# nfrasser/lasgun

Hardware: NVIDIA B200
Metric: Mrays/s (primary+shadow) (higher is better)
Workload: dtype f64

## Files before the change

lasgun_b200/csrc/lgb_kernels.cu:

```cuda
#include <math_constants.h>

#include <algorithm>

#include "lgb_math.cuh"

namespace lgb {

template <class T> __device__ __forceinline__ void wst(T* p, T v) { __stcs(p, v); }
template <class T> __device__ __forceinline__ T wld(const T* p) { return __ldcs(p); }

struct RayF {
    float ox, oy, oz;
    float ix, iy, iz;
    float nx, ny, nz;
    float dx, dy, dz;
    float inv_dd, inv_len;
    float sx, sy, sz;
    float err;
    int kz;
    unsigned oct;
};

__device__ __forceinline__ float clamp_idir(float d) {
    const float v = 1.0f / d;
// ... 1286 lines not shown
        const unsigned long long v0 = __popc(__ballot_sync(0xFFFFFFFFu, primary != 0)), v1 = __popc(__ballot_sync(0xFFFFFFFFu, hits != 0));
        if (lane == 0) { atomicAdd(&ctr(O)->primary_rays, v0); atomicAdd(&ctr(O)->primary_hits, v1); }
        if (STATS) {
            for (int k = 0; k < 3; k++) {
                unsigned long long a = warp_sum(lc.filter[k]), b = warp_sum(lc.exact[k]);
                if (lane == 0) { atomicAdd(&ctr(O)->filter[k], a); atomicAdd(&ctr(O)->exact[k], b); atomicAdd(&ctr(O)->p_filter[k], a); atomicAdd(&ctr(O)->p_exact[k], b); }
            }
        }
    }
}

template <bool ALL_SHADOWS, bool INST, bool RAYBUF = false>
__global__ void __launch_bounds__(kAppendThreads) k_setup(DevScene S, DevCamera C, DevShade sh, DevWork W, DevOut O, DevWave V) {
    constexpr bool LEAN = !INST && !RAYBUF;
    const uint64_t total = W.n_pixels * W.spp;
    const uint64_t g = (uint64_t)blockIdx.x * blockDim.x + threadIdx.x;
    uint32_t need = 0;
    bool live = false;
    if (g < total) {
        const uint32_t ref = V.hit_ref[g];
        const double t_hit = V.hit_t[g];
        Ray64 ray; uint32_t x, y, s;
        bool ref_done = false;
        if (ref != kSlotUnused && slot_ray<RAYBUF>(C, W, g, ray, x, y, s)) {
            const uint64_t gi = ((uint64_t)y * W.w + x) * W.spp + s;
            if (ref == LGB_MISS) {
                if (O.aov_id) O.aov_id[gi] = LGB_MISS;
                if (O.aov_t) O.aov_t[gi] = CUDART_INF;
                if (O.aov_occl) O.aov_occl[gi] = 0;
            } else {
                if (!ALL_SHADOWS && S.specular && (material_flags(S, ref) & kMatSpecular)) { V.occl[g] = 0; V.gate[g] = 0; ref_done = true; }
            }
            if (ref != LGB_MISS && !ref_done) {
                live = true;
                const double t = t_hit;
                D3 ng, ps; double wo_ng; uint32_t sflags = kSfGeneric;
                if (LEAN) {
                    LeanSurf Ls;
                    lean_surface<true>(S, ray, t, ref, 0u, Ls);
                    sflags = Ls.flags;
                    if (!(sflags & kSfGeneric)) {
                        ng = (sflags & kSfNgFlip) ? -Ls.n : Ls.n;
                        ps = ray.o + ray.d * t + ng * (2.220446049250313e-16 * 65536.0);
                        wo_ng = 1.0;
                    }
                }
                if (sflags & kSfGeneric) {
                    ShadePoint P; uint32_t id;
                    shade_point<false, INST>(S, ray, t, ref, P, id);
                    ng = P.ng; ps = P.ps; wo_ng = dot(P.wo, P.ng);
                }
                V.ps[3 * g + 0] = ps.x; V.ps[3 * g + 1] = ps.y; V.ps[3 * g + 2] = ps.z;
                if (O.aov_id) O.aov_id[gi] = canonical_id(S, ref);
                if (O.aov_t) O.aov_t[gi] = t;
                const uint32_t gate = light_gates(S, ray, ps, ng, wo_ng, !(sflags & kSfGeneric));
                need = ALL_SHADOWS ? (S.n_lights >= 32u ? 0xFFFFFFFFu : (1u << S.n_lights) - 1u) : gate;
                V.occl[g] = 0;
                V.gate[g] = gate;
                if (LEAN) V.sflags[g] = (unsigned char)sflags;
            }
        }
    }
    if (S.grids) return;
    __shared__ MultiAppendScratch sc;
    __shared__ uint32_t qmap[2 * LGB_MAX_LIGHTS];
    if (threadIdx.x < 2 * S.n_lights) qmap[threadIdx.x] = (threadIdx.x >> 1) * 3 + ((threadIdx.x & 1) ? kQueueB : kQueueA);
    __syncthreads();
    const bool anchor = W.spp == 1 || (uint32_t)g - fdiv((uint32_t)g, W.fd_spp) * W.spp == W.anchor;
    unsigned long long flags = 0;
    if (live) for (uint32_t l = 0; l < S.n_lights; l++) if ((need >> l) & 1u) flags |= 1ull << (2 * l + (anchor ? 0 : 1));
    block_append_multi(sc, 2 * S.n_lights, flags, (uint32_t)g, V.queue, V.queue_stride, V.queue_count, qmap);
}

template <bool INST>
__device__ __forceinline__ bool occludes(const DevScene& S, uint32_t ref, const Ray64& world) {
    const uint32_t type = ref >> 30, idx = ref & 0x3FFFFFFFu;
    Ray64 ray = world;
    if (INST) ray = ray_to_space(S, space_of(S, ref), world);
    double t;
    if (type == LGB_PRIM_TRIANGLE) {
        const float4* tp = S.tri + 3 * (size_t)idx;
        const float4 q0 = __ldg(tp), q1 = __ldg(tp + 1), q2 = __ldg(tp + 2);
        double b0, b1, b2;
        return triangle_exact(d3(q0.x, q0.y, q0.z), d3(q1.x, q1.y, q1.z), d3(q2.x, q2.y, q2.z), ray, t, b0, b1, b2) && t < 1.0;
    }
    if (type == LGB_PRIM_SPHERE) {
        const double2 c01 = __ldg(reinterpret_cast<const double2*>(S.sph64 + 4 * (size_t)idx));
        const double2 c23 = __ldg(reinterpret_cast<const double2*>(S.sph64 + 4 * (size_t)idx + 2));
        bool inside;
        return sphere_exact(d3(c01.x, c01.y, c23.x), c23.y, ray, t, inside) && t < 1.0;
    }
    double mn[3], mx[3];
#pragma unroll
    for (int k = 0; k < 3; k++) { mn[k] = __ldg(&S.cub64[6 * (size_t)idx + k]); mx[k] = __ldg(&S.cub64[6 * (size_t)idx + 3 + k]); }
    int ua, va;
    return cuboid_exact(mn, mx, ray, t, ua, va) && t < 1.0;
}

#ifndef LGB_PRETEST_ITEMS
#define LGB_PRETEST_ITEMS 2
#endif
constexpr int kPretestItems = LGB_PRETEST_ITEMS;
template <bool INST>
__global__ void __launch_bounds__(kAppendThreads) k_pretest(DevScene S, DevWork W, DevOut O, DevWave V, uint32_t light) {
    __shared__ AppendScratch sc;
    const unsigned total = V.queue_count[light * 3 + kQueueB];
    const unsigned lane = threadIdx.x & 31u;
    const double* L = S.lights + 9 * (size_t)light;
    const D3 lp = d3(L[0], L[1], L[2]);
    unsigned ncached = 0;
    for (uint64_t i0 = (uint64_t)blockIdx.x * blockDim.x * kPretestItems; i0 < total; i0 += (uint64_t)gridDim.x * blockDim.x * kPretestItems) {
        const uint64_t first = i0 + threadIdx.x * kPretestItems;
        uint32_t g[kPretestItems], oc[kPretestItems];
        unsigned to_c = 0;
#pragma unroll
        for (int k = 0; k < kPretestItems; k++) {
            g[k] = 0; oc[k] = LGB_MISS;
            if (first + k < total) {
                g[k] = V.queue[(size_t)(light * 3 + kQueueB) * V.queue_stride + first + k];
                if (g[k] != kEntryDone) {
                    oc[k] = V.occluder[(size_t)light * W.n_pixels + fdiv(g[k], W.fd_spp)];
                    to_c |= 1u << k;
                }
            }
        }
#pragma unroll
        for (int k = 0; k < kPretestItems; k++) {
            if (oc[k] != LGB_MISS) {
                Ray64 ray;
                ray.o = d3(V.ps[3 * (size_t)g[k]], V.ps[3 * (size_t)g[k] + 1], V.ps[3 * (size_t)g[k] + 2]);
                ray.d = lp - ray.o;
                if (occludes<INST>(S, oc[k], ray)) { atomicOr(&V.occl[g[k]], 1u << light); to_c &= ~(1u << k); ncached++; }
            }
        }
        block_append_n<kPretestItems>(sc, to_c, g, V.queue + (size_t)(light * 3 + kQueueC) * V.queue_stride, &V.queue_count[light * 3 + kQueueC]);
    }
    if (O.counters) {
        const unsigned long long n = warp_sum(ncached);
        if (lane == 0 && n) { atomicAdd(&ctr(O)->shadow_cached, n); atomicAdd(&ctr(O)->shadow_occluded, n); }
        if (blockIdx.x == 0 && threadIdx.x == 0) atomicAdd(&ctr(O)->shadow_traced, (unsigned long long)total);
    }
}

#ifndef LGB_SBEAM_THREADS
#define LGB_SBEAM_THREADS_ 64
#else
#define LGB_SBEAM_THREADS_ LGB_SBEAM_THREADS
#endif
template <bool STATS>
__global__ void __launch_bounds__(LGB_SBEAM_THREADS_, 1024 / LGB_SBEAM_THREADS_) k_sbeam(DevScene S, DevWork W, DevOut O, DevWave V, uint32_t light,
                                                                                     uint2* list_out, uint32_t* count_out) {
    const unsigned total = V.free_count[light];
    const unsigned i = blockIdx.x * blockDim.x + threadIdx.x;
    const unsigned lane = threadIdx.x & 31u;
    LocalCounters lc = {};
    if (i < total) {
        const uint32_t ga = V.queue[(size_t)(light * 3 + kQueueC) * V.queue_stride + i];
        const uint32_t p = fdiv(ga, W.fd_spp);
        {
        const double* Lp = S.lights + 9 * (size_t)light;
        const D3 lp = d3(Lp[0], Lp[1], Lp[2]);
        Ray64 centre; centre.o = lp;
        centre.d = d3(V.ps[3 * (size_t)ga], V.ps[3 * (size_t)ga + 1], V.ps[3 * (size_t)ga + 2]) - lp;
        double dmin[3] = {centre.d.x, centre.d.y, centre.d.z}, dmax[3] = {centre.d.x, centre.d.y, centre.d.z};
        for (uint32_t k = 0; k < W.spp; k++) {
            const size_t g = (size_t)p * W.spp + k;
            const uint32_t ref = V.hit_ref[g];
            if (ref == LGB_MISS || ref == kSlotUnused) continue;
            const double dx = V.ps[3 * g] - lp.x, dy = V.ps[3 * g + 1] - lp.y, dz = V.ps[3 * g + 2] - lp.z;
            dmin[0] = fmin(dmin[0], dx); dmax[0] = fmax(dmax[0], dx); dmin[1] = fmin(dmin[1], dy); dmax[1] = fmax(dmax[1], dy);
            dmin[2] = fmin(dmin[2], dz); dmax[2] = fmax(dmax[2], dz);
        }
        const double dc[3] = {centre.d.x, centre.d.y, centre.d.z};
        float sp[3];
        for (int a = 0; a < 3; a++) {
            if (!(dmin[a] > 0.0) && !(dmax[a] < 0.0)) { sp[a] = 1e30f; continue; }
            const double lo = fmin(fabs(dmin[a]), fabs(dmax[a])), hi = fmax(fabs(dmin[a]), fabs(dmax[a])), c = fabs(dc[a]);
            const double up = c / lo - 1.0, dn = 1.0 - c / hi;
            sp[a] = __double2float_ru(fmax(fmax(up, dn), 0.0) * 1.0000001 + 4e-7);
        }
        BeamF B; B.sx = sp[0]; B.sy = sp[1]; B.sz = sp[2];
        const RayF f = make_rayf(centre, S.err_abs);
        const float smax = 1.0f + 1e-5f;
        uint32_t stack[kStackDepth]; int sp_ = 0;
        uint2 list[kBeamList];
        uint32_t n = 0, cur = 0;
        bool over = false;
        while (cur != kDone && !over) {
            if (cur & kLeafBit) {
                const uint32_t type = (cur >> 29) & 3u, count = ((cur >> 24) & 31u) + 1u, first = cur & kLeafFirstMask;
                for (uint32_t k = 0; k < count; k++) {
                    const uint32_t idx = first + k;
                    float lx, ly, lz, hx, hy, hz;
                    if (type == LGB_PRIM_TRIANGLE) {
                        const float4* tp = S.tri + 3 * (size_t)idx;
                        const float4 q0 = __ldg(tp), q1 = __ldg(tp + 1), q2 = __ldg(tp + 2);
                        lx = fminf(q0.x, fminf(q1.x, q2.x)); hx = fmaxf(q0.x, fmaxf(q1.x, q2.x));
                        ly = fminf(q0.y, fminf(q1.y, q2.y)); hy = fmaxf(q0.y, fmaxf(q1.y, q2.y));
                        lz = fminf(q0.z, fminf(q1.z, q2.z)); hz = fmaxf(q0.z, fmaxf(q1.z, q2.z));
                    } else if (type == LGB_PRIM_SPHERE) {
                        const float4 s4 = __ldg(&S.sph32[idx]);
                        const float rr = __fadd_ru(s4.w, f.err);
                        lx = __fsub_rd(s4.x, rr); hx = __fadd_ru(s4.x, rr); ly = __fsub_rd(s4.y, rr); hy = __fadd_ru(s4.y, rr); lz = __fsub_rd(s4.z, rr); hz = __fadd_ru(s4.z, rr);
                    } else {
                        const float4 lo = __ldg(&S.cub32[2 * idx]), hi = __ldg(&S.cub32[2 * idx + 1]);
                        lx = lo.x; ly = lo.y; lz = lo.z; hx = hi.x; hy = hi.y; hz = hi.z;
                    }
                    if (type != LGB_PRIM_CUBOID) {
                        lx = __fsub_rd(lx, f.err); ly = __fsub_rd(ly, f.err); lz = __fsub_rd(lz, f.err);
                        hx = __fadd_ru(hx, f.err); hy = __fadd_ru(hy, f.err); hz = __fadd_ru(hz, f.err);
                    }
                    float tn;
                    if (!beam_slab<8>(lx, ly, lz, hx, hy, hz, f, B, tn) || tn > smax) continue;
                    if (n == (uint32_t)kBeamList) { over = true; break; }
                    list[n++] = make_uint2(kLeafBit | (type << 29) | idx, __float_as_uint(tn));
                }
                cur = kDone;
            } else {
                const float4* np = S.nodes + 4 * (size_t)cur;
                const float4 n0 = __ldg(np), n1 = __ldg(np + 1), n2 = __ldg(np + 2);
                const float2 n3 = __ldg(reinterpret_cast<const float2*>(np + 3));
                if (STATS) lc.node_tests++;
                float t0, t1;
                bool h0, h1;
                switch (f.oct) {
#define LGB_BEAM_CASE(o) case o: h0 = beam_slab<o>(n0.x, n0.y, n0.z, n0.w, n1.x, n1.y, f, B, t0); h1 = beam_slab<o>(n1.z, n1.w, n2.x, n2.y, n2.z, n2.w, f, B, t1); break;
                LGB_BEAM_CASE(0) LGB_BEAM_CASE(1) LGB_BEAM_CASE(2) LGB_BEAM_CASE(3) LGB_BEAM_CASE(4) LGB_BEAM_CASE(5) LGB_BEAM_CASE(6)
                default: h0 = beam_slab<7>(n0.x, n0.y, n0.z, n0.w, n1.x, n1.y, f, B, t0); h1 = beam_slab<7>(n1.z, n1.w, n2.x, n2.y, n2.z, n2.w, f, B, t1); break;
#undef LGB_BEAM_CASE
                }
                h0 = h0 && t0 <= smax; h1 = h1 && t1 <= smax;
                const uint32_t c0 = __float_as_uint(n3.x), c1 = __float_as_uint(n3.y);
                if (h0 && h1) { cur = c0; stack[sp_++] = c1; }
                else if (h0) cur = c0;
                else if (h1) cur = c1;
                else cur = kDone;
            }
            if (cur == kDone && sp_ && !over) cur = stack[--sp_];
        }
        if (!over) {
            for (uint32_t k = 0; k < n; k++) list_out[(size_t)k * W.n_pixels + p] = list[k];
            count_out[p] = n;
        }
        }
    }
    if (O.counters && STATS) {
        unsigned long long nt = warp_sum(lc.node_tests);
        if (lane == 0) atomicAdd(&ctr(O)->node_tests, nt);
    }
}
#ifndef LGB_SWALK_THREADS
#define LGB_SWALK_THREADS 128
#endif
#ifndef LGB_SBEAM_THREADS
#define LGB_SBEAM_THREADS 64
#endif
template <bool STATS>
__global__ void __launch_bounds__(LGB_SWALK_THREADS, 1024 / LGB_SWALK_THREADS) k_swalk(DevScene S, DevWork W, DevOut O, DevWave V, uint32_t light,
                                                                                       const uint2* list_in, const uint32_t* count_in) {
    const unsigned total = V.queue_count[light * 3 + kQueueB];
    const unsigned i = blockIdx.x * blockDim.x + threadIdx.x;
    const unsigned lane = threadIdx.x & 31u;
    LocalCounters lc = {};
    unsigned occluded = 0;
    if (i < total) {
        uint32_t* slot = V.queue + (size_t)(light * 3 + kQueueB) * V.queue_stride + i;
        const uint32_t g = *slot;
        const uint32_t p = fdiv(g, W.fd_spp);
        const uint32_t n = count_in[p];
        if (n != kBeamOverflow) {
            const double* Lp = S.lights + 9 * (size_t)light;
            Ray64 world;
            world.o = d3(V.ps[3 * (size_t)g], V.ps[3 * (size_t)g + 1], V.ps[3 * (size_t)g + 2]);
            world.d = d3(Lp[0], Lp[1], Lp[2]) - world.o;
            Ray64 ray; RayF f; Trav T;
            enter_root<false>(S, world, ray, f, T, 1.0);
            bool hit = false;
            for (uint32_t k = 0; k < n && !hit; k++) {
                const uint2 e = __ldg(&list_in[(size_t)k * W.n_pixels + p]);
                hit = leaf_prims<true, STATS, false>(S, world, ray, f, T, (e.x >> 29) & 3u, 1u, e.x & kLeafFirstMask, 1.0, lc);
            }
            if (hit) { atomicOr(&V.occl[g], 1u << light); occluded++; }
            *slot = kEntryDone;
        }
    }
    if (O.counters) {
        unsigned long long v = warp_sum(occluded);
        if (lane == 0 && v) atomicAdd(&ctr(O)->shadow_occluded, v);
        if (STATS) {
            for (int k = 0; k < 3; k++) {
                unsigned long long a = warp_sum(lc.filter[k]), b = warp_sum(lc.exact[k]);
                if (lane == 0) { atomicAdd(&ctr(O)->filter[k], a); atomicAdd(&ctr(O)->exact[k], b); }
            }
        }
    }
}

#ifndef LGB_GSHADOW_THREADS
#define LGB_GSHADOW_THREADS 64
#endif
#ifndef LGB_GSHADOW_MIN_BLOCKS
#define LGB_GSHADOW_MIN_BLOCKS (1536 / LGB_GSHADOW_THREADS)
#endif
template <bool STATS>
__device__ __forceinline__ bool grid_blocked(const DevScene& S, D3 o, uint32_t l, LocalCounters& lc) {
    Ray64 world;
    world.o = o;
    const double* Lp = S.lights + 9 * (size_t)l;
    world.d = d3(Lp[0], Lp[1], Lp[2]) - world.o;
    const double ax = fabs(world.d.x), ay = fabs(world.d.y), az = fabs(world.d.z);
    const int a = ax >= ay ? (ax >= az ? 0 : 2) : (ay >= az ? 1 : 2);
    const double da = -(a == 0 ? world.d.x : a == 1 ? world.d.y : world.d.z);
    const double db = -(a == 0 ? world.d.y : a == 1 ? world.d.z : world.d.x), dc = -(a == 0 ? world.d.z : a == 1 ? world.d.x : world.d.y);
    if (da == 0.0) return false;
    const DevGrid* G = S.grids + l;
    const uint32_t res = __ldg(&G->res), n_large = __ldg(&G->n_large);
    const int face = 2 * a + (da < 0.0 ? 1 : 0);
    const double* map = G->map[face];
    const double inv = fast_rcp(fabs(da));
    const int cu = min(max((int)floor((db * inv - __ldg(map)) * __ldg(map + 1)), 0), (int)res - 1);
    const int cv = min(max((int)floor((dc * inv - __ldg(map + 2)) * __ldg(map + 3)), 0), (int)res - 1);
    const size_t cell = ((size_t)face * res + (size_t)cv) * res + (size_t)cu;
    const uint32_t* cs = G->cell_start;
    const uint32_t b = __ldg(cs + cell), e = __ldg(cs + cell + 1);
    Ray64 ray; RayF f; Trav T;
    enter_root<false>(S, world, ray, f, T, 1.0);
    const float dd = f.dx * f.dx + f.dy * f.dy + f.dz * f.dz;
    const float len_up = dd * f.inv_len * (1.0f + 1e-5f) + f.err;
    bool hit = false;
    const bool sorted = e - b <= kGridSortMax;
    const uint2* en = G->entries;
    const uint2* lg = G->large;
    for (uint32_t i = b; i < e && !hit; i++) {
        const uint2 r = __ldg(en + i);
        if (__uint_as_float(r.y) > len_up) { if (sorted) break; else continue; }
        hit = leaf_prims<true, STATS, false>(S, world, ray, f, T, r.x >> 30, 1u, r.x & 0x3FFFFFFFu, 1.0, lc);
    }
    for (uint32_t i = 0; i < n_large && !hit; i++) {
        const uint2 r = __ldg(lg + i);
        if (__uint_as_float(r.y) > len_up) break;
        hit = leaf_prims<true, STATS, false>(S, world, ray, f, T, r.x >> 30, 1u, r.x & 0x3FFFFFFFu, 1.0, lc);
    }
    return hit;
}

template <bool STATS, bool ALL_SHADOWS>
__global__ void __launch_bounds__(LGB_GSHADOW_THREADS, LGB_GSHADOW_MIN_BLOCKS) k_gshadow(DevScene S, DevCamera C, DevWork W, DevOut O, DevWave V) {
    const uint64_t total = W.n_pixels * W.spp;
    const uint64_t g = (uint64_t)blockIdx.x * blockDim.x + threadIdx.x;
    const unsigned lane = threadIdx.x & 31u;
    LocalCounters lc = {};
    unsigned traced = 0, occluded = 0;
    if (g < total) {
        const uint32_t ref = wld(&V.hit_ref[g]);
        uint32_t mask = 0;
        D3 ps = d3(0, 0, 0);
        const uint32_t gate = ALL_SHADOWS ? (S.n_lights >= 32u ? 0xFFFFFFFFu : (1u << S.n_lights) - 1u) : wld(&V.gate[g]);
        ps = d3(wld(&V.ps[3 * g]), wld(&V.ps[3 * g + 1]), wld(&V.ps[3 * g + 2]));
        if (ref != LGB_MISS && ref != kSlotUnused) mask = gate;
        if (mask) {
            uint32_t occl = 0;
            for (uint32_t l = 0; l < S.n_lights; l++) {
                if (!((mask >> l) & 1u)) continue;
                traced++;
                if (grid_blocked<STATS>(S, ps, l, lc)) { occl |= 1u << l; occluded++; }
            }
            wst(&V.occl[g], occl);
        }
    }
    if (O.counters) {
        const unsigned long long v0 = warp_sum(traced), v1 = warp_sum(occluded);
        if (lane == 0 && v0) {
            if (W.mode == 3) atomicAdd(&ctr(O)->secondary_rays, v0);
            else { atomicAdd(&ctr(O)->shadow_traced, v0); atomicAdd(&ctr(O)->shadow_occluded, v1); }
        }
        if (STATS) {
            for (int k = 0; k < 3; k++) {
                unsigned long long a = warp_sum(lc.filter[k]), b = warp_sum(lc.exact[k]);
                if (lane == 0) { atomicAdd(&ctr(O)->filter[k], a); atomicAdd(&ctr(O)->exact[k], b); }
            }
        }
    }
}

template <bool STATS, bool INST>
__global__ void __launch_bounds__(LGB_TRAV_THREADS, LGB_MIN_BLOCKS) k_shadow(DevScene S, DevWork W, DevOut O, DevWave V, uint32_t light, int which) {
    const unsigned total = V.queue_count[light * 3 + which];
    const uint32_t* q = V.queue + (size_t)(light * 3 + which) * V.queue_stride;
    const bool record = which == kQueueA && W.spp > 1;
    const double* L = S.lights + 9 * (size_t)light;
    const D3 lp = d3(L[0], L[1], L[2]);
    const unsigned lane = threadIdx.x & 31u;
    LocalCounters lc = {};
    unsigned int occluded = 0;
    uint32_t stack[kStackDepth];
    Ray64 world, ray; RayF f; Trav T;
    uint32_t g = 0;
    bool active = false, drained = false;
    for (;;) {
        if (!drained) {
            const unsigned idle = __ballot_sync(0xFFFFFFFFu, !active);
            if (idle == 0xFFFFFFFFu) {
                const unsigned long long idx = warp_fetch(V.queue_fetch + light * 3 + which, !active, lane);
                if (!active && idx < total) {
                    g = q[idx];
                    world.o = d3(V.ps[3 * (size_t)g], V.ps[3 * (size_t)g + 1], V.ps[3 * (size_t)g + 2]);
                    world.d = lp - world.o;
                    enter_root<INST>(S, world, ray, f, T, 1.0); active = true;
                }
                drained = __any_sync(0xFFFFFFFFu, idx != ~0ull && idx >= total);
            }
        }
        const unsigned amask = __ballot_sync(0xFFFFFFFFu, active);
        if (!amask) break;
        const unsigned oct0 = __shfl_sync(0xFFFFFFFFu, f.oct, __ffs(amask) - 1);
        const unsigned octw = __all_sync(0xFFFFFFFFu, !active || f.oct == oct0) ? oct0 : 8u;
        if (active) {
            const bool done = trav_run<true, STATS, true, INST>(S, world, ray, f, T, stack, nullptr, 1.0, lc, 0, octw);
            if (done) {
                if (T.best.ref != LGB_MISS) { atomicOr(&V.occl[g], 1u << light); occluded++; }
                if (record) V.occluder[(size_t)light * W.n_pixels + fdiv(g, W.fd_spp)] = T.best.ref;
                if (record && W.beams && T.best.ref == LGB_MISS) {
                    const unsigned peers = __activemask(), leader = __ffs(peers) - 1;
                    uint32_t base = 0;
                    if (lane == leader) base = atomicAdd(V.free_count + light, (uint32_t)__popc(peers));
                    base = __shfl_sync(peers, base, leader);
                    V.queue[(size_t)(light * 3 + kQueueC) * V.queue_stride + base + __popc(peers & ((1u << lane) - 1u))] = g;
                }
                active = false;
            }
        }
    }
    if (O.counters) {
        unsigned long long v = warp_sum(occluded);
        if (lane == 0) atomicAdd(&ctr(O)->shadow_occluded, v);
        if (which == kQueueA && blockIdx.x == 0 && threadIdx.x == 0) atomicAdd(&ctr(O)->shadow_traced, (unsigned long long)total);
        if (STATS) {
            unsigned long long n = warp_sum(lc.node_tests);
            if (lane == 0) atomicAdd(&ctr(O)->node_tests, n);
            for (int k = 0; k < 3; k++) {
                unsigned long long a = warp_sum(lc.filter[k]), b = warp_sum(lc.exact[k]);
                if (lane == 0) { atomicAdd(&ctr(O)->filter[k], a); atomicAdd(&ctr(O)->exact[k], b); }
            }
        }
    }
}

#ifndef LGB_SHADE_MIN_BLOCKS
#define LGB_SHADE_MIN_BLOCKS 4
#endif
#ifndef LGB_FUSED_THREADS
#define LGB_FUSED_THREADS 128u
#endif
#ifndef LGB_GSHADE_MIN_BLOCKS
#define LGB_GSHADE_MIN_BLOCKS 2
#endif
__device__ __forceinline__ uchar4 quantise(D3 c) {
    uchar4 px;
    px.x = (unsigned char)round(fmin(fmax(c.x, 0.0), 1.0) * 255.0);
    px.y = (unsigned char)round(fmin(fmax(c.y, 0.0), 1.0) * 255.0);
    px.z = (unsigned char)round(fmin(fmax(c.z, 0.0), 1.0) * 255.0);
    px.w = 255;
    return px;
}
__device__ __forceinline__ void spawn_children(const ShadePoint& P, const DevWave& V, uint32_t g) {
    SpawnRec rec; rec.slot = g; rec.child_r = rec.child_t = kNoChild; rec.pad = 0;
    rec.spec_r[0] = rec.spec_r[1] = rec.spec_r[2] = rec.spec_t[0] = rec.spec_t[1] = rec.spec_t[2] = rec.c = 0.0;
    Ray64 rr, rt; D3 spec, wi;
    bool has_r = false, has_t = false;
    if (sample_specular_reflection(P.B, spec, wi) && !(spec.x == 0.0 && spec.y == 0.0 && spec.z == 0.0) && !(dot(wi, P.ns) <= 0.0)) {
        has_r = true; rr.o = P.ps; rr.d = -1.0 * P.wo + 2.0 * dot(P.wo, P.ns) * P.ns;
        rec.spec_r[0] = spec.x; rec.spec_r[1] = spec.y; rec.spec_r[2] = spec.z;
    }
    if (sample_specular_transmission(P.B, spec, wi)) {
        const double c = fabs(dot(wi, P.ns));
        if (!(spec.x == 0.0 && spec.y == 0.0 && spec.z == 0.0) && c != 0.0) {
            has_t = true; rt.o = P.pt; rt.d = wi; rec.c = c;
            rec.spec_t[0] = spec.x; rec.spec_t[1] = spec.y; rec.spec_t[2] = spec.z;
        }
    }
    const unsigned peers = __activemask(), lane = threadIdx.x & 31u, leader = __ffs(peers) - 1;
    const unsigned mr = __ballot_sync(peers, has_r), mt = __ballot_sync(peers, has_t);
    uint32_t b_rec = 0, b_r = 0, b_t = 0;
    if (lane == leader) {
        b_rec = atomicAdd(V.spawn_ctr, (uint32_t)__popc(peers));
        if (mr) b_r = atomicAdd(V.spawn_ctr + 1, (uint32_t)__popc(mr));
        if (mt) b_t = atomicAdd(V.spawn_ctr + 2, (uint32_t)__popc(mt));
    }
    b_rec = __shfl_sync(peers, b_rec, leader); b_r = __shfl_sync(peers, b_r, leader); b_t = __shfl_sync(peers, b_t, leader);
    const unsigned below = (1u << lane) - 1u;
    if (has_r) {
        rec.child_r = b_r + __popc(mr & below);
        double* o = V.next_rays + 6 * (size_t)rec.child_r; o[0] = rr.o.x; o[1] = rr.o.y; o[2] = rr.o.z; o[3] = rr.d.x; o[4] = rr.d.y; o[5] = rr.d.z;
    }
    if (has_t) {
        rec.child_t = V.next_t_base + b_t + __popc(mt & below);
        double* o = V.next_rays + 6 * (size_t)rec.child_t; o[0] = rt.o.x; o[1] = rt.o.y; o[2] = rt.o.z; o[3] = rt.d.x; o[4] = rt.d.y; o[5] = rt.d.z;
    }
    V.recs[b_rec + __popc(peers & below)] = rec;
}

template <bool INST, bool FUSED, bool GENERAL = false, bool RAYBUF = false>
__global__ void __launch_bounds__(256, GENERAL ? LGB_GSHADE_MIN_BLOCKS : LGB_SHADE_MIN_BLOCKS) k_shade(DevScene S, DevCamera C, DevShade sh, DevWork W, DevOut O, DevWave V) {
    const double PI = 3.14159265358979323846264338327950288;
    const uint64_t total = W.n_pixels * W.spp;
    __shared__ double rad[FUSED ? 256 * 3 : 3];
    __shared__ unsigned char valid[FUSED ? 256 : 1];
    uint64_t g;
    bool mine;
    if (FUSED) {
        const uint32_t ppb = blockDim.x / W.spp;
        const uint64_t p = (uint64_t)blockIdx.x * ppb + threadIdx.x / W.spp;
        mine = threadIdx.x < ppb * W.spp && p < W.n_pixels;
        g = p * W.spp + threadIdx.x % W.spp;
    } else {
        g = (uint64_t)blockIdx.x * blockDim.x + threadIdx.x;
        mine = g < total;
    }
    D3 output = d3(0, 0, 0);
    bool have = false;
    uint32_t x = 0, y = 0, s = 0;
    if (mine) {
        const uint32_t ref = V.hit_ref[g];
        Ray64 ray;
        if (ref != kSlotUnused && slot_ray<RAYBUF>(C, W, g, ray, x, y, s)) {
            have = true;
            if (ref == LGB_MISS) {
                output = background_of(sh, ray.d);
            } else {
                ShadePoint P; uint32_t id;
                shade_point<true, INST, GENERAL>(S, ray, V.hit_t[g], ref, P, id);
                const bool general = GENERAL && (P.B.flags & kMatGeneral);
                if (GENERAL && (P.B.flags & kMatSpecular) && W.depth < S.recursion && V.recs) spawn_children(P, V, (uint32_t)g);
                else if (GENERAL && (P.B.flags & kMatSpecular) && W.depth < S.recursion) {
                    const unsigned peers = __activemask();
                    const unsigned lane = threadIdx.x & 31u, leader = __ffs(peers) - 1;
                    uint32_t base = 0;
                    if (lane == leader) base = atomicAdd(V.sec_count, (uint32_t)__popc(peers));
                    base = __shfl_sync(peers, base, leader);
                    V.sec_list[base + __popc(peers & ((1u << lane) - 1u))] = (uint32_t)g;
                }
                const uint32_t occl = V.occl[g];
                if (O.aov_occl) O.aov_occl[((uint64_t)y * W.w + x) * W.spp + s] = occl;
                for (uint32_t l = 0; l < S.n_lights; l++) {
                    if ((occl >> l) & 1u) continue;
                    const double* L = S.lights + 9 * (size_t)l;
                    D3 wi = d3(L[0], L[1], L[2]) - P.ps;
                    double dist = sqrt(dot(wi, wi));
                    double f_att = L[6] + L[7] * dist + L[8] * dist * dist;
                    if (f_att == 0.0) continue;
                    wi = wi * (1.0 / dist);
                    double wi_dot_n = dot(wi, P.ns);
                    D3 f = general ? bsdf_f_general(P.B, wi) : bsdf_f(P.B, wi);
                    output = output + mul_el(PI * d3(L[3], L[4], L[5]), f) * wi_dot_n / f_att;
                }
                output = output + mul_el(d3(sh.ambient[0], sh.ambient[1], sh.ambient[2]), general ? bsdf_f_general(P.B, P.ns) : bsdf_f(P.B, P.ns));
                D3 zero = d3(0, 0, 0);
                output = output + zero + zero;
            }
        }
    }
    if (!FUSED) {
        if (have) { O.radiance[3 * g + 0] = output.x; O.radiance[3 * g + 1] = output.y; O.radiance[3 * g + 2] = output.z; }
        return;
    }
    rad[3 * threadIdx.x] = output.x; rad[3 * threadIdx.x + 1] = output.y; rad[3 * threadIdx.x + 2] = output.z;
    valid[threadIdx.x] = have ? 1 : 0;
    __syncthreads();
    if (mine && threadIdx.x % W.spp == 0 && valid[threadIdx.x]) {
        D3 c = d3(0, 0, 0);
        for (uint32_t k = 0; k < W.spp; k++) c = c + d3(rad[3 * (threadIdx.x + k)], rad[3 * (threadIdx.x + k) + 1], rad[3 * (threadIdx.x + k) + 2]);
        c = c * (1.0 / (double)W.spp);
        const uint64_t p = (uint32_t)g / W.spp;
        reinterpret_cast<uchar4*>(O.film)[W.compact_out ? W.compact_base + p : (uint64_t)y * W.w + x] = quantise(c);
    }
}

struct LeanHit { D3 wo, ns; double woz, cos_o, Ao, alpha2; bool glossy; };
__device__ __forceinline__ void lean_eval(const LeanHit& H, D3 wi, double wn, double f_att, double& a, double& g) {
    const double PI = 3.14159265358979323846264338327950288;
    g = 0.0;
    const double cos_i = fabs(wn);
    if (H.glossy && cos_i != 0.0) {
        const double u = 1.0 + fdot(wi, H.wo);
        const double z = wn + H.woz, z2 = z * z;
        if (u > 0.0 && z2 != 0.0) {
            const double twou = u + u;
            const double Q = fma(H.alpha2, z2, fmax(twou - z2, 0.0));
            const double c = fmin(fast_sqrt(0.5 * u), 1.0);
            const double cos_t = fast_sqrt(fmax(fma(fma(c, c, -1.0), 4.0 / 9.0, 1.0), 0.0));
            const double ta = fma(1.5, c, -cos_t), tb = fma(1.5, c, cos_t), tc = fma(-1.5, cos_t, c), td = fma(1.5, cos_t, c);
            const double ad = ta * td, cb = tc * tb, bd = tb * td;
            const double fnum = fma(ad, ad, cb * cb), fden = 2.0 * (bd * bd);
            const double Ai = fast_sqrt(fma(H.alpha2, fmax(fma(-cos_i, cos_i, 1.0), 0.0), cos_i * cos_i));
            const double K = PI * (Q * Q) * (2.0 * fma(H.Ao, cos_i, Ai * H.cos_o)) * fden;
            if (K > 0.0) {
                const double R = fast_rcp(K * f_att);
                g = H.alpha2 * fnum * (twou * twou) * R * wn;
                a = wn * K * R;
                return;
            }
        }
    }
    a = wn * fast_rcp(f_att);
}

__device__ __forceinline__ D3 lean_radiance(const DevScene& S, const DevShade& sh, const Ray64& ray, double t, const LeanSurf& Ls, uint32_t sflags, uint32_t lit) {
    const double PI = 3.14159265358979323846264338327950288;
    D3 output = d3(0, 0, 0);
    LeanHit H;
    H.ns = (sflags & kSfNsFlip) ? -Ls.n : Ls.n;
    const D3 ng = (sflags & kSfNgFlip) ? -Ls.n : Ls.n;
    const D3 ps = fmadd(ng, 2.220446049250313e-16 * 65536.0, fmadd(ray.d, t, ray.o));
    H.wo = ray.d * -fast_rsqrt(fdot(ray.d, ray.d));
    H.woz = fdot(H.wo, H.ns); H.cos_o = fabs(H.woz);
    const double* M = S.materials + kMatStride * (size_t)Ls.material;
    const uint32_t mflags = (uint32_t)__double_as_longlong(M[7]);
    H.glossy = mflags & kMatGlossy; H.alpha2 = M[3] * M[3];
    H.Ao = H.glossy ? fast_sqrt(fma(H.alpha2, fmax(fma(-H.cos_o, H.cos_o, 1.0), 0.0), H.cos_o * H.cos_o)) : 0.0;
    if (H.woz != 0.0) {
        D3 dsum = d3(0, 0, 0), gsum = d3(0, 0, 0);
        for (uint32_t l = 0; l < S.n_lights; l++) {
            if (!((lit >> l) & 1u)) continue;
            const double* L = S.lights + 9 * (size_t)l;
            const D3 v = d3(L[0], L[1], L[2]) - ps;
            const double d2 = fdot(v, v);
            if (!(d2 > 0.0)) continue;
            const double inv = fast_rsqrt(d2), dist = d2 * inv;
            const double f_att = fma(L[8] * dist, dist, fma(L[7], dist, L[6]));
            if (f_att == 0.0) continue;
            const D3 wi = v * inv;
            double a, gl;
            lean_eval(H, wi, fdot(wi, H.ns), f_att, a, gl);
            const D3 I = PI * d3(L[3], L[4], L[5]);
            dsum = fmadd(I, a, dsum); gsum = fmadd(I, gl, gsum);
        }
        if (((sflags & kSfNsFlip) != 0) == ((sflags & kSfNgFlip) != 0)) {
            double a, gl;
            lean_eval(H, H.ns, 1.0, 1.0, a, gl);
            const D3 amb = d3(sh.ambient[0], sh.ambient[1], sh.ambient[2]);
            dsum = fmadd(amb, a, dsum); gsum = fmadd(amb, gl, gsum);
        }
        const double inv_pi = 0.318309886183790671537767526745028724;
        const D3 kd = (mflags & kMatDiffuse) ? d3(M[0], M[1], M[2]) * inv_pi : d3(0, 0, 0);
        output = d3(fma(kd.x, dsum.x, M[4] * gsum.x), fma(kd.y, dsum.y, M[5] * gsum.y), fma(kd.z, dsum.z, M[6] * gsum.z));
    }
    return output;
}

__device__ __forceinline__ D3 shade_generic_plastic(const DevScene& S, const DevShade& sh, const Ray64& ray, double t, uint32_t ref, uint32_t occl) {
    const double PI = 3.14159265358979323846264338327950288;
    ShadePoint P; uint32_t id;
    shade_point<true, false, false>(S, ray, t, ref, P, id);
    D3 output = d3(0, 0, 0);
    for (uint32_t l = 0; l < S.n_lights; l++) {
        if ((occl >> l) & 1u) continue;
        const double* L = S.lights + 9 * (size_t)l;
        D3 wi = d3(L[0], L[1], L[2]) - P.ps;
        const double dist = sqrt(dot(wi, wi));
        const double f_att = L[6] + L[7] * dist + L[8] * dist * dist;
        if (f_att == 0.0) continue;
        wi = wi * (1.0 / dist);
        const double wi_dot_n = dot(wi, P.ns);
        output = output + mul_el(PI * d3(L[3], L[4], L[5]), bsdf_f(P.B, wi)) * wi_dot_n / f_att;
    }
    return output + mul_el(d3(sh.ambient[0], sh.ambient[1], sh.ambient[2]), bsdf_f(P.B, P.ns));
}

#ifndef LGB_LEAN_MIN_BLOCKS
// ... 507 lines not shown
```

Baseline: 25630.

## Specialize grid shadow test with lean float ray state and recompute-on-demand

Replaces the general enter_root/leaf_prims path in the grid shadow test with a dedicated per-primitive routine that keeps only a small float ray struct live. The double-precision ray is re-read from memory when an exact test is needed instead of being held in registers. Light iteration now walks set bits with ffs/popc, and the shadow point is prefetched into L1. The aim is lower register pressure and higher occupancy in the shadow kernel, paid for with extra loads and recomputation after each exact miss.

```diff
diff --git a/lasgun_b200/csrc/lgb_kernels.cu b/lasgun_b200/csrc/lgb_kernels.cu
--- a/lasgun_b200/csrc/lgb_kernels.cu
+++ b/lasgun_b200/csrc/lgb_kernels.cu
@@ -1612,19 +1612,109 @@
 #ifndef LGB_GSHADOW_MIN_BLOCKS
 #define LGB_GSHADOW_MIN_BLOCKS (1536 / LGB_GSHADOW_THREADS)
 #endif
+struct ShadowF { float ox, oy, oz, dx, dy, dz, inv_dd, inv_len, err, len_up; };
+__device__ __forceinline__ ShadowF shadow_f(const Ray64& r, float err_abs) {
+    ShadowF f;
+    f.ox = (float)r.o.x; f.oy = (float)r.o.y; f.oz = (float)r.o.z;
+    f.dx = (float)r.d.x; f.dy = (float)r.d.y; f.dz = (float)r.d.z;
+    const float dd = f.dx * f.dx + f.dy * f.dy + f.dz * f.dz;
+    f.inv_dd = 1.0f / dd;
+    f.inv_len = rsqrtf(dd);
+    f.err = (dd > 1e-24f && dd < 1e24f) ? err_abs : CUDART_INF_F;
+    f.len_up = dd * f.inv_len * (1.0f + 1e-5f) + f.err;
+    return f;
+}
+
+__device__ __forceinline__ Ray64 gshadow_ray(const double* ps, const double* Lp) {
+    Ray64 r;
+    r.o = d3(__ldg(ps), __ldg(ps + 1), __ldg(ps + 2));
+    r.d = d3(__ldg(Lp), __ldg(Lp + 1), __ldg(Lp + 2)) - r.o;
+    return r;
+}
+
+__device__ __forceinline__ float gshadow_here(float v) { asm volatile("" : "+f"(v)); return v; }
+
+__device__ __forceinline__ int gshadow_kz(const ShadowF& f, const double* ps, const double* Lp) {
+    const float x = fabsf(gshadow_here(f.dx)), y = fabsf(gshadow_here(f.dy)), z = fabsf(gshadow_here(f.dz));
+    if (x == y || x == z || y == z) return max_dimension_abs(gshadow_ray(ps, Lp).d);
+    return x > y ? (x > z ? 0 : 2) : (y > z ? 1 : 2);
+}
+
+enum GShadowResult { kGsFiltered, kGsMissed, kGsBlocked };
 template <bool STATS>
-__device__ __forceinline__ bool grid_blocked(const DevScene& S, D3 o, uint32_t l, LocalCounters& lc) {
-    Ray64 world;
-    world.o = o;
+__device__ __forceinline__ GShadowResult gshadow_prim(const DevScene& S, const ShadowF& f, const double* ps, const double* Lp, uint32_t type,
+                                                      uint32_t idx, LocalCounters& lc) {
+    double t;
+    bool hit;
+    if (type == LGB_PRIM_TRIANGLE) {
+        const float4* tp = S.tri + 3 * (size_t)idx;
+        const float4 q0 = __ldg(tp), q1 = __ldg(tp + 1), q2 = __ldg(tp + 2);
+        if (STATS) lc.filter[2]++;
+        RayF r;
+        r.ox = f.ox; r.oy = f.oy; r.oz = f.oz; r.err = f.err;
+        r.kz = gshadow_kz(f, ps, Lp);
+        const int kx = (r.kz + 1) % 3, ky = (kx + 1) % 3;
+        const float dx = gshadow_here(f.dx), dy = gshadow_here(f.dy), dz = gshadow_here(f.dz);
+        float fdz = r.kz == 0 ? dx : (r.kz == 1 ? dy : dz);
+        float fdx = kx == 0 ? dx : (kx == 1 ? dy : dz);
+        float fdy = ky == 0 ? dx : (ky == 1 ? dy : dz);
+        r.sz = 1.0f / fdz;
+        r.sx = -fdx * r.sz;
+        r.sy = -fdy * r.sz;
+        const bool pass = r.kz == 0 ? tri_filter<0>(q0, q1, q2, r, 1.0f) : r.kz == 1 ? tri_filter<1>(q0, q1, q2, r, 1.0f) : tri_filter<2>(q0, q1, q2, r, 1.0f);
+        if (!pass) return kGsFiltered;
+        if (STATS) lc.exact[2]++;
+        double b0, b1, b2;
+        hit = triangle_exact(d3(q0.x, q0.y, q0.z), d3(q1.x, q1.y, q1.z), d3(q2.x, q2.y, q2.z), gshadow_ray(ps, Lp), t, b0, b1, b2);
+    } else if (type == LGB_PRIM_SPHERE) {
+        const float4 s = __ldg(&S.sph32[idx]);
+        if (STATS) lc.filter[0]++;
+        float lx = s.x - f.ox, ly = s.y - f.oy, lz = s.z - f.oz;
+        float bq = lx * f.dx + ly * f.dy + lz * f.dz;
+        float tc = bq * f.inv_dd;
+        float wx = __fmaf_rn(-tc, f.dx, lx), wy = __fmaf_rn(-tc, f.dy, ly), wz = __fmaf_rn(-tc, f.dz, lz);
+        float perp2 = wx * wx + wy * wy + wz * wz;
+        float rr = s.w + 2.0f * f.err;
+        if (perp2 > rr * rr * (1.0f + 1e-6f)) return kGsFiltered;
+        float half = rr * f.inv_len;
+        float slack = fabsf(tc) * 2e-6f + 2.0f * f.err * f.inv_len;
+        if (tc - half - slack > 1.0f) return kGsFiltered;
+        if (tc + half + slack < 0.0f) return kGsFiltered;
+        if (STATS) lc.exact[0]++;
+        const double2 c01 = __ldg(reinterpret_cast<const double2*>(S.sph64 + 4 * (size_t)idx));
+        const double2 c23 = __ldg(reinterpret_cast<const double2*>(S.sph64 + 4 * (size_t)idx + 2));
+        bool inside;
+        hit = sphere_exact(d3(c01.x, c01.y, c23.x), c23.y, gshadow_ray(ps, Lp), t, inside);
+    } else {
+        const float4 lo = __ldg(&S.cub32[2 * idx]), hi = __ldg(&S.cub32[2 * idx + 1]);
+        if (STATS) lc.filter[1]++;
+        RayF r;
+        r.ix = clamp_idir(gshadow_here(f.dx)); r.iy = clamp_idir(gshadow_here(f.dy)); r.iz = clamp_idir(gshadow_here(f.dz));
+        r.nx = -f.ox * r.ix; r.ny = -f.oy * r.iy; r.nz = -f.oz * r.iz;
+        float tn;
+        if (!slab2(lo.x, lo.y, lo.z, hi.x, hi.y, hi.z, r, CUDART_INF_F, tn)) return kGsFiltered;
+        if (STATS) lc.exact[1]++;
+        double mn[3], mx[3];
+#pragma unroll
+        for (int k = 0; k < 3; k++) { mn[k] = __ldg(&S.cub64[6 * (size_t)idx + k]); mx[k] = __ldg(&S.cub64[6 * (size_t)idx + 3 + k]); }
+        int ua, va;
+        hit = cuboid_exact(mn, mx, gshadow_ray(ps, Lp), t, ua, va);
+    }
+    return hit && t < 1.0 ? kGsBlocked : kGsMissed;
+}
+
+template <bool STATS>
+__device__ __forceinline__ bool grid_blocked(const DevScene& S, const double* ps, uint32_t l, LocalCounters& lc) {
     const double* Lp = S.lights + 9 * (size_t)l;
-    world.d = d3(Lp[0], Lp[1], Lp[2]) - world.o;
-    const double ax = fabs(world.d.x), ay = fabs(world.d.y), az = fabs(world.d.z);
+    const Ray64 ray = gshadow_ray(ps, Lp);
+    const D3 d = ray.d;
+    const double ax = fabs(d.x), ay = fabs(d.y), az = fabs(d.z);
     const int a = ax >= ay ? (ax >= az ? 0 : 2) : (ay >= az ? 1 : 2);
-    const double da = -(a == 0 ? world.d.x : a == 1 ? world.d.y : world.d.z);
-    const double db = -(a == 0 ? world.d.y : a == 1 ? world.d.z : world.d.x), dc = -(a == 0 ? world.d.z : a == 1 ? world.d.x : world.d.y);
+    const double da = -(a == 0 ? d.x : a == 1 ? d.y : d.z);
+    const double db = -(a == 0 ? d.y : a == 1 ? d.z : d.x), dc = -(a == 0 ? d.z : a == 1 ? d.x : d.y);
     if (da == 0.0) return false;
     const DevGrid* G = S.grids + l;
-    const uint32_t res = __ldg(&G->res), n_large = __ldg(&G->n_large);
+    const uint32_t res = __ldg(&G->res);
     const int face = 2 * a + (da < 0.0 ? 1 : 0);
     const double* map = G->map[face];
     const double inv = fast_rcp(fabs(da));
@@ -1633,25 +1723,24 @@
     const size_t cell = ((size_t)face * res + (size_t)cv) * res + (size_t)cu;
     const uint32_t* cs = G->cell_start;
     const uint32_t b = __ldg(cs + cell), e = __ldg(cs + cell + 1);
-    Ray64 ray; RayF f; Trav T;
-    enter_root<false>(S, world, ray, f, T, 1.0);
-    const float dd = f.dx * f.dx + f.dy * f.dy + f.dz * f.dz;
-    const float len_up = dd * f.inv_len * (1.0f + 1e-5f) + f.err;
-    bool hit = false;
-    const bool sorted = e - b <= kGridSortMax;
-    const uint2* en = G->entries;
-    const uint2* lg = G->large;
-    for (uint32_t i = b; i < e && !hit; i++) {
-        const uint2 r = __ldg(en + i);
-        if (__uint_as_float(r.y) > len_up) { if (sorted) break; else continue; }
-        hit = leaf_prims<true, STATS, false>(S, world, ray, f, T, r.x >> 30, 1u, r.x & 0x3FFFFFFFu, 1.0, lc);
-    }
-    for (uint32_t i = 0; i < n_large && !hit; i++) {
-        const uint2 r = __ldg(lg + i);
-        if (__uint_as_float(r.y) > len_up) break;
-        hit = leaf_prims<true, STATS, false>(S, world, ray, f, T, r.x >> 30, 1u, r.x & 0x3FFFFFFFu, 1.0, lc);
-    }
-    return hit;
+    ShadowF f = shadow_f(ray, S.err_abs);
+    const uint2* en = G->entries + b;
+    uint32_t n = e - b;
+    bool cell_list = true, skip_far = n > kGridSortMax;
+    for (;;) {
+        if (n == 0) {
+            if (!cell_list) return false;
+            cell_list = false; skip_far = false;
+            en = G->large; n = __ldg(&G->n_large);
+            continue;
+        }
+        const uint2 r = __ldg(en);
+        en++; n--;
+        if (__uint_as_float(r.y) > f.len_up) { if (!skip_far) n = 0; continue; }
+        const GShadowResult k = gshadow_prim<STATS>(S, f, ps, Lp, r.x >> 30, r.x & 0x3FFFFFFFu, lc);
+        if (k == kGsBlocked) return true;
+        if (k == kGsMissed) f = shadow_f(gshadow_ray(ps, Lp), S.err_abs);
+    }
 }
 
 template <bool STATS, bool ALL_SHADOWS>
@@ -1664,17 +1753,19 @@
     if (g < total) {
         const uint32_t ref = wld(&V.hit_ref[g]);
         uint32_t mask = 0;
-        D3 ps = d3(0, 0, 0);
-        const uint32_t gate = ALL_SHADOWS ? (S.n_lights >= 32u ? 0xFFFFFFFFu : (1u << S.n_lights) - 1u) : wld(&V.gate[g]);
-        ps = d3(wld(&V.ps[3 * g]), wld(&V.ps[3 * g + 1]), wld(&V.ps[3 * g + 2]));
+        const uint32_t lights = S.n_lights >= 32u ? 0xFFFFFFFFu : (1u << S.n_lights) - 1u;
+        const uint32_t gate = ALL_SHADOWS ? lights : wld(&V.gate[g]);
+        const double* ps = V.ps + 3 * g;
+        asm volatile("prefetch.global.L1 [%0];" :: "l"(ps));
         if (ref != LGB_MISS && ref != kSlotUnused) mask = gate;
         if (mask) {
             uint32_t occl = 0;
-            for (uint32_t l = 0; l < S.n_lights; l++) {
-                if (!((mask >> l) & 1u)) continue;
-                traced++;
-                if (grid_blocked<STATS>(S, ps, l, lc)) { occl |= 1u << l; occluded++; }
-            }
+            traced = __popc(mask & lights);
+            for (uint32_t todo = mask & lights; todo; todo &= todo - 1u) {
+                const uint32_t l = __ffs(todo) - 1;
+                if (grid_blocked<STATS>(S, ps, l, lc)) occl |= 1u << l;
+            }
+            occluded = __popc(occl);
             wst(&V.occl[g], occl);
         }
     }
```

Result: faster. 27700, median of 6 (+8.1%).
